# sakdag/multimodal-misinformation-detection

Measured on AMD Instinct MI355X. Metric: claim–evidence pairs/sec (fwd+bwd) at bs=256; 1/2/4/8 MI355X scaling, higher is better.
Workload: dtype fp32; 1 GPU; full fine-tune bert-base-uncased + ViT-B/16 + fusion head (768/768, E=256, H=8), fwd+bwd+AdamW; global_batch=256, seq_len=128, image_size=224, parallelism=dp1

## Files before the change

multimodal-misinformation-detection_amd/csrc/attention.hip:

```cpp
#include "attn_common.h"
#include "attn_stream.h"
#include "attn_resident.h"
#include "attn_split.h"
#include <algorithm>
#include <initializer_list>
#include <stdio.h>
#include <stdlib.h>
#include <string.h>

namespace {

int g_v2_generic = [] {
  const char* v = getenv("MMFD_ATTN_V2_GENERIC");
  return v && atoi(v) != 0 ? 1 : 0;
}();

const bool g_attn_v1 = getenv("MMFD_ATTN_V1") != nullptr;

int g_fp32_attn_mode = [] {
  const char* v = getenv("MMFD_FP32_ATTN");
  const char* gm = getenv("MMFD_FP32_GEMM");
  const bool native = (v && (!strcmp(v, "native") || !strcmp(v, "0"))) ||
                      (!v && gm && (!strcmp(gm, "native") || !strcmp(gm, "0")));
  return native ? 0 : 1;
}();

const int g_x6a_dbg = getenv("MMFD_X6A_DBG") ? atoi(getenv("MMFD_X6A_DBG")) : 0;

int fill(const mmfd_attn_args& a, AttnP& p, bool bwd) {
  MMFD_CHECK_ARG(a.dtype == MMFD_F32 || a.dtype == MMFD_BF16, "attn: bad dtype");
  MMFD_CHECK_ARG(a.D > 0 && a.D <= 64, "attn: head_dim %lld unsupported (<= 64)", (long long)a.D);
  MMFD_CHECK_ARG(a.B >= 0 && a.H > 0 && a.Lq >= 0 && a.Lk > 0, "attn: bad shape");
  MMFD_CHECK_ARG(a.q && a.k && a.v && a.o && a.lse, "attn: null pointer");
  const int epc = a.dtype == MMFD_BF16 ? 8 : 4;
  MMFD_CHECK_ARG(a.D % epc == 0, "attn: head_dim*element_size must be a multiple of 16 bytes");
  auto al = [&](const void* ptr, int64_t sb, int64_t st) {
    return ((uintptr_t)ptr & 15) == 0 && sb % epc == 0 && st % epc == 0;
  };
  MMFD_CHECK_ARG(al(a.q, a.q_sb, a.q_st) && al(a.k, a.k_sb, a.k_st) && al(a.v, a.v_sb, a.v_st),
                 "attn: q/k/v must be 16-B aligned with strides multiple of 16 B");
  MMFD_CHECK_ARG(a.dropout_p <= 0.f || a.seed, "attn: dropout needs seed");
  MMFD_CHECK_ARG(a.dropout_p < 1.f, "attn: dropout p must be < 1");
  if (bwd) {
    MMFD_CHECK_ARG(a.dout && a.dq && a.dk && a.dv && a.delta, "attn_bwd: null pointer");
    MMFD_CHECK_ARG(al(a.dout, a.do_sb, a.do_st), "attn_bwd: dout alignment");
    if (a.d_rel_bias) {
      MMFD_CHECK_ARG(a.rel_bias && a.rel_bias_sb == a.H * a.Lq * a.Lk && a.rel_bias_mod == 0,
                     "attn_bwd: d_rel_bias needs a per-batch rel_bias [B][H][Lq][Lk] (rel_bias_sb = H*Lq*Lk, rel_bias_mod = 0)");
// ... 83 lines not shown
  return KERN_TD(attn_fwd_v2_kernel, HPB, false, 0);
}

template <typename T, int D, bool REL, int MODE>
void add_bwd_v2(Plan& pl, AttnP& p, const char* what) {
  constexpr int NTH = V2T<T>::DKDV_THREADS;
  const int lq_pad = v2_pad(p.Lq, v2_kc<T>()), lk_pad = v2_pad(p.Lk, v2_kc<T>());
  constexpr int dkdv_max = v2_dkdv_lds<T, D>(V2_LMAX, V2_LMAX / 32);
  p.dm_lds = p.p > 0.f && p.dm && v2_dkdv_lds<T, D>(lq_pad, p.dmw) <= dkdv_max;
  const dim3 heads((unsigned)(p.B * p.H));
  pl.add(KERN_TD(attn_dq_v2_kernel, REL, MODE), heads, V2_THREADS, v2_dq_lds<T, D>(lk_pad), v2_dq_lds<T, D>(V2_LMAX), what);
  pl.add(KERN_TD(attn_dkdv_v2_kernel, NTH, REL, MODE), heads, NTH, v2_dkdv_lds<T, D>(lq_pad, p.dm_lds ? p.dmw : 0),
         dkdv_max, what);
}

template <typename T, int D>
void plan_kernels(Plan& pl, AttnP& p, const mmfd_attn_args& a, bool bwd) {
  const char* what = bwd ? "attn_bwd" : "attn_fwd";
  const int64_t nbh = p.B * p.H;
  const dim3 heads((unsigned)nbh);
  const dim3 qblocks((unsigned)((p.Lq + 63) / 64), (unsigned)nbh), kblocks((unsigned)((p.Lk + 63) / 64), (unsigned)nbh);
  if (pl.family == SPLIT) {
    const int lq16 = v2_pad(p.Lq, 16), lk16 = v2_pad(p.Lk, 16);
    if (!bwd) {
      pl.add(p.p > 0.f ? KERN_D(attn_fwd_x6_kernel, true) : KERN_D(attn_fwd_x6_kernel, false), heads, V2_THREADS,
             x6_kv_lds(lk16), X6A_LDS, what);
    } else {
      const int dqd = p.p <= 0.f ? 0 : !p.dm ? 1 : 2;
      const int dkd = dqd == 2 && x6_dkdv_lds(lq16, lk16, p.dmw) > X6A_LDS_MAX ? 1 : dqd;
      pl.add(dqd == 0 ? KERN_D(attn_dq_x6_kernel, 0) : dqd == 1 ? KERN_D(attn_dq_x6_kernel, 1) : KERN_D(attn_dq_x6_kernel, 2),
             heads, V2_THREADS, x6_kv_lds(lk16), X6A_LDS, what);
      pl.add(dkd == 0 ? KERN_D(attn_dkdv_x6_kernel, 0) : dkd == 1 ? KERN_D(attn_dkdv_x6_kernel, 1) : KERN_D(attn_dkdv_x6_kernel, 2),
             heads, V2_THREADS, x6_dkdv_lds(lq16, lk16, dkd == 2 ? p.dmw : 0), X6A_LDS_MAX, what);
    }
  } else if (pl.family == RESIDENT && !bwd) {
    const int hpb = p.Lk <= 64 && p.Lq <= 32 ? 4 : p.Lk <= 64 && p.Lq <= 64 ? 2 : 1;
    const int lmax = hpb > 1 ? 64 : sizeof(T) == 2 ? V2_LMAX_FWD : V2_LMAX;
    pl.add(hpb == 4 ? fwd_v2_kern<T, D, 4>(p) : hpb == 2 ? fwd_v2_kern<T, D, 2>(p) : fwd_v2_kern<T, D, 1>(p),
           dim3((unsigned)((nbh + hpb - 1) / hpb)), V2_THREADS,
           v2_fwd_lds<T, D>(hpb, v2_pad(p.Lk, v2_kc<T>())) + (p.cos_ls ? v2_fwd_cos_lds(hpb, v2_pad(p.Lk, v2_kc<T>())) : 0),
           v2_fwd_lds<T, D>(hpb, lmax) + v2_fwd_cos_lds(hpb, lmax), what);
  } else if (pl.family == RESIDENT) {
    const int mode = v2_mode(p);
    if (p.rel_bias) add_bwd_v2<T, D, true, 0>(pl, p, what);
    else if (mode == 1) add_bwd_v2<T, D, false, 1>(pl, p, what);
    else if (mode == 2) add_bwd_v2<T, D, false, 2>(pl, p, what);
    else add_bwd_v2<T, D, false, 0>(pl, p, what);
  } else if (!bwd) {
    pl.add(KERN_TD(attn_fwd_kernel), qblocks, 256, stream_kv_lds<T, D>(), 0, what);
  } else {
    const int64_t threads = nbh * p.Lq * AT<T, D>::NCH;
    pl.add(KERN_TD(attn_delta_kernel), dim3((unsigned)((threads + 255) / 256)), 256, 0, 0, what);
    pl.add(KERN_TD(attn_bwd_dkdv_kernel), kblocks, 256, stream_dkdv_lds<T, D>(), 0, what);
    pl.add(KERN_TD(attn_bwd_dq_kernel), qblocks, 256, stream_dq_lds<T, D>(), 0, what);
// ... 92 lines not shown
    const Step& st = pl.step[i];
    put("%s", st.k.name);
    for (int j = 0; j < st.k.narg; ++j) {
      if (j == 0) put("%s", st.k.bf < 0 ? "<" : st.k.bf ? "<bf16," : "<float,");
      put(j + 1 < st.k.narg ? "%d," : "%d>", st.k.arg[j]);
    }
    put(" grid=%u,%u,%u block=%u lds=%d%s%s%s%s%s%s", st.grid.x, st.grid.y, st.grid.z, st.block, st.lds,
        p.pl ? " pl" : "", p.pl_only ? " pl_only" : "", p.vst ? " vst" : "", p.dm ? " dm" : "",
        p.dm_lds ? " dm_lds" : "", p.idx32 ? " idx32" : "");
    if (p.pl) put(" pl_stride=%lld", (long long)p.pl_stride);
    put("%s", "\n");
  }
  if (pl.split3) put("mmfd_split3 rows=%lld W=%lld\n", (long long)(p.B * p.Lq), (long long)((bwd ? 3 : 1) * a->H * a->D));
  MMFD_CHECK_ARG(at < bytes, "mmfd_debug_attn_plan: buffer of %lld bytes is too small", (long long)bytes);
  return 0;
}

extern "C" int mmfd_debug_set_attn_v2_generic(int on) {
  const int old = g_v2_generic;
  g_v2_generic = on ? 1 : 0;
  return old;
}

extern "C" int mmfd_set_fp32_attn_mode(int mode) {
  MMFD_CHECK_ARG(mode == 0 || mode == 1, "mmfd_set_fp32_attn_mode: mode %d (0 = fp32 MFMA, 1 = split operands)", mode);
  const int old = g_fp32_attn_mode;
  g_fp32_attn_mode = mode;
  return old;
}

#ifdef MMFD_X6A_STAMPS
extern "C" int mmfd_debug_x6a_stamps(void* host_dst, int64_t bytes) {
  return (int)hipMemcpyFromSymbol(host_dst, HIP_SYMBOL(x6a_stamps), (size_t)bytes, 0, hipMemcpyDeviceToHost);
}
#endif
```

multimodal-misinformation-detection_amd/csrc/attn_split.h:

```cpp
#pragma once
#include "attn_resident.h"

namespace {


#ifdef MMFD_X6A_STAMPS
__device__ uint64_t x6a_stamps[8192 * 8 * 16];
#define X6A_STAMP(k)                                                                               \
  do {                                                                                             \
    const uint64_t t__ = __builtin_amdgcn_s_memtime();                                             \
    if (lane == 0 && blockIdx.x < 8192) x6a_stamps[((int64_t)blockIdx.x * 8 + wave) * 16 + (k)] = t__; \
  } while (0)
#else
#define X6A_STAMP(k) do { } while (0)
#endif
constexpr int X6A_LMAX = 208;
constexpr int X6A_RB = 128;
constexpr int X6A_LDS = 6 * X6A_LMAX * X6A_RB + 3 * X6A_LMAX * 4;
constexpr int X6A_LDS_MAX = 160 * 1024;
constexpr int x6_kv_lds(int lk16) { return 6 * lk16 * X6A_RB + lk16 * 4; }
constexpr int x6_dkdv_lds(int lq16, int lk16, int dm_words) {
  return 6 * lq16 * X6A_RB + (2 * lq16 + lk16) * 4 + lq16 * dm_words * 4;
}

__device__ __forceinline__ void split8(const float* x, uint4& hi, uint4& mid, uint4& lo) {
  bf16x8 h, m, l;
#pragma unroll
  for (int u = 0; u < 8; ++u) {
    const bf16 hu = (bf16)x[u];
    const float r = x[u] - (float)hu;
    const bf16 mu = (bf16)r;
    h[u] = hu;
    m[u] = mu;
    l[u] = (bf16)(r - (float)mu);
// ... 15 lines not shown

__device__ __forceinline__ void split_acc(const f32x4& a, const f32x4& b, uint4& hi, uint4& mid, uint4& lo) {
  const float x[8] = {a[0], a[1], a[2], a[3], b[0], b[1], b[2], b[3]};
  split8(x, hi, mid, lo);
}

template <int KCH> struct X6Row { float4 v[KCH][2]; };
template <int KCH>
__device__ __forceinline__ void x6_row_load(X6Row<KCH>& x, const float* __restrict__ base, int64_t st, int64_t row,
                                            int64_t nrows, int lane, int dreal) {
  const int g = lane >> 4;
#pragma unroll
  for (int kc = 0; kc < KCH; ++kc) {
    const int col = (kc * 4 + g) * 8;
    x.v[kc][0] = x.v[kc][1] = make_float4(0.f, 0.f, 0.f, 0.f);
    if (row < nrows && col < dreal) {
      const float* src = base + row * st + col;
      x.v[kc][0] = *reinterpret_cast<const float4*>(src);
      x.v[kc][1] = *reinterpret_cast<const float4*>(src + 4);
    }
  }
}
template <int KCH>
__device__ __forceinline__ void x6_row_split(uint4 (&f)[3][KCH], const X6Row<KCH>& x) {
#pragma unroll
  for (int kc = 0; kc < KCH; ++kc) {
    const float4 a = x.v[kc][0], b = x.v[kc][1];
    const float e[8] = {a.x, a.y, a.z, a.w, b.x, b.y, b.z, b.w};
    split8(e, f[0][kc], f[1][kc], f[2][kc]);
  }
}

template <int D, int NTH>
__device__ __forceinline__ void x6_stage2(char* img_a, const float* __restrict__ base_a, int64_t st_a, char* img_b,
                                          const float* __restrict__ base_b, int64_t st_b, int img, int64_t nrows,
                                          int nrows_pad, int tid, int dreal, int dbg) {
  constexpr int NC = D / 8;
  constexpr int MAXT = (X6A_LMAX * NC + NTH - 1) / NTH;
  const int total = nrows_pad * NC;
  float4 xa[MAXT][2], xb[MAXT][2];
#pragma unroll
  for (int j = 0; j < MAXT; ++j) {
    const int c = tid + j * NTH;
    const int r = c / NC, ch = c % NC;
    xa[j][0] = xa[j][1] = xb[j][0] = xb[j][1] = make_float4(0.f, 0.f, 0.f, 0.f);
    if (c < total && r < nrows && ch * 8 < dreal && !(dbg & 1)) {
      const float* sa = base_a + (int64_t)r * st_a + ch * 8;
      const float* sb = base_b + (int64_t)r * st_b + ch * 8;
      xa[j][0] = *reinterpret_cast<const float4*>(sa);
      xa[j][1] = *reinterpret_cast<const float4*>(sa + 4);
      xb[j][0] = *reinterpret_cast<const float4*>(sb);
      xb[j][1] = *reinterpret_cast<const float4*>(sb + 4);
    }
  }
#pragma unroll
  for (int j = 0; j < MAXT; ++j) {
    const int c = tid + j * NTH;
    if (c < total) {
      const int r = c / NC, ch = c % NC;
      const int off = row_off<bf16, 64>(r, ch);
      uint4 h, m, l;
      {
        const float e[8] = {xa[j][0].x, xa[j][0].y, xa[j][0].z, xa[j][0].w, xa[j][1].x, xa[j][1].y, xa[j][1].z, xa[j][1].w};
        split8(e, h, m, l);
        *reinterpret_cast<uint4*>(img_a + off) = h;
        *reinterpret_cast<uint4*>(img_a + img + off) = m;
        *reinterpret_cast<uint4*>(img_a + 2 * img + off) = l;
      }
      {
        const float e[8] = {xb[j][0].x, xb[j][0].y, xb[j][0].z, xb[j][0].w, xb[j][1].x, xb[j][1].y, xb[j][1].z, xb[j][1].w};
        split8(e, h, m, l);
        *reinterpret_cast<uint4*>(img_b + off) = h;
        *reinterpret_cast<uint4*>(img_b + img + off) = m;
        *reinterpret_cast<uint4*>(img_b + 2 * img + off) = l;
      }
    }
  }
}

__device__ __forceinline__ uint4 x6_tr_frag(const char* lds, int c, int dsub, int lane, int h1off) {
  const int g = lane >> 4, i = lane & 15, q = i >> 2;
  const int u = dsub * 4 + (i & 3);
  const int r = c * 32 + 4 * g + q;
  const int off = r * X6A_RB + (((u >> 1) ^ (r & 7)) << 4) + ((u & 1) << 3);
  const uint2 x0 = lds_read_tr16(lds + off);
  const uint2 x1 = lds_read_tr16(lds + off + h1off);
  return make_uint4(x0.x, x0.y, x1.x, x1.y);
}

__device__ __forceinline__ void x6_row_frag3(uint4* f, const char* lds, int img, int sub, int kc, int lane) {
  f[0] = row_frag<bf16, 64>(lds, sub, kc, lane);
  f[1] = row_frag<bf16, 64>(lds + img, sub, kc, lane);
  f[2] = row_frag<bf16, 64>(lds + 2 * img, sub, kc, lane);
}
__device__ __forceinline__ void x6_tr_frag3(uint4* f, const char* lds, int img, int c, int d, int lane, int h1off) {
  f[0] = x6_tr_frag(lds, c, d, lane, h1off);
  f[1] = x6_tr_frag(lds + img, c, d, lane, h1off);
  f[2] = x6_tr_frag(lds + 2 * img, c, d, lane, h1off);
}


template <int D, bool DROP>
__global__ void __launch_bounds__(V2_THREADS, 1) attn_fwd_x6_kernel(AttnP p) {
  constexpr int KCH = D / 32, DT = D / 16;
  extern __shared__ __attribute__((aligned(16))) char smem[];
  const int tid = threadIdx.x, lane = tid & 63, g = lane >> 4, li = lane & 15;
  const int wave = __builtin_amdgcn_readfirstlane(tid >> 6);
  const int64_t bh = blockIdx.x, b = bh / p.H, h = bh % p.H;
  X6A_STAMP(0);
  const int lk16 = v2_pad(p.Lk, 16);
  const int img = lk16 * X6A_RB;
  char* k_img = smem;
  char* v_img = smem + 3 * img;
  float* kbias = reinterpret_cast<float*>(smem + 6 * img);
  const float* qb = reinterpret_cast<const float*>(p.q) + b * p.q_sb + h * p.D;
  X6Row<KCH> qn;
  x6_row_load<KCH>(qn, qb, p.q_st, (int64_t)wave * 16 + li, p.Lq, lane, p.D);
  x6_stage2<D, V2_THREADS>(k_img, reinterpret_cast<const float*>(p.k) + b * p.k_sb + h * p.D, p.k_st, v_img,
                           reinterpret_cast<const float*>(p.v) + b * p.v_sb + h * p.D, p.v_st, img, p.Lk, lk16, tid,
                           p.D, p.dbg);
  stage_kbias<V2_THREADS>(kbias, p, b, lk16, tid);
  __syncthreads();
  X6A_STAMP(1);
  const uint64_t seed = DROP ? *p.seed : 0ull;
  const uint32_t hkey = mmfd_hash_key(seed, p.salt);
  const float c2 = p.scale * LOG2E;
  float* ob = reinterpret_cast<float*>(p.o) + b * p.o_sb + h * p.D;
  const int nqb = (int)((p.Lq + 15) / 16);
  const int nfc = lk16 / 64;
  const int nchk = nfc + ((lk16 & 63) ? 1 : 0);
  auto qrun = [&](int qbk, const uint4 (&qf)[3][KCH], int c0, int c1, f32x4 (&o)[DT], float& m, float& lsum) {
// ... 101 lines not shown
  auto qfin = [&](int qbk, const f32x4 (&o)[DT], float m, float lsum) {
    const int64_t q0 = (int64_t)qbk * 16, myq = q0 + li;
#pragma unroll
    for (int r = 0; r < 4; ++r) {
      const float lr = __shfl(lsum, 4 * g + r, 64);
      const int64_t q = q0 + 4 * g + r;
      const float inv = 1.0f / lr;
      if (q < p.Lq) {
#pragma unroll
        for (int d = 0; d < DT; ++d)
          if (d * 16 + li < p.D) {
            const float val = o[d][r] * inv;
            ob[q * p.o_st + d * 16 + li] = val;
            if (p.pl) plane_put(p, ob + q * p.o_st + d * 16 + li, val);
          }
      }
    }
    if (g == 0 && myq < p.Lq) p.lse[bh * p.Lq + myq] = (m + log2f(lsum)) * LN2;
  };
  if (p.dbg & 2) return;
  const int R = nqb - V2_THREADS / 64;
  const bool split = R >= 1 && R <= V2_THREADS / 64 && (R & 3) == 1 && nchk >= 2;
  const int nwhole = split ? nqb - 1 : nqb;
  for (int qbk = wave; qbk < nwhole; qbk += V2_THREADS / 64) {
    uint4 qf[3][KCH];
    x6_row_split<KCH>(qf, qn);
    if (qbk + V2_THREADS / 64 < nwhole)
      x6_row_load<KCH>(qn, qb, p.q_st, (int64_t)(qbk + V2_THREADS / 64) * 16 + li, p.Lq, lane, p.D);
    if (qbk == wave) X6A_STAMP(2);
    float m = -INFINITY, lsum = 0.f;
    f32x4 o[DT];
#pragma unroll
    for (int d = 0; d < DT; ++d) o[d] = f32x4{0.f, 0.f, 0.f, 0.f};
    qrun(qbk, qf, 0, nchk, o, m, lsum);
    if (qbk == wave) X6A_STAMP(7);
    lsum += __shfl_xor(lsum, 16, 64);
    lsum += __shfl_xor(lsum, 32, 64);
    qfin(qbk, o, m, lsum);
    if (qbk == wave) X6A_STAMP(8);
  }
  if (split) {
    const int sb = nqb - 1, hc = nchk / 2;
    const bool own = wave == R - 1, part = wave == R;
    float m = -INFINITY, lsum = 0.f;
    f32x4 o[DT];
#pragma unroll
    for (int d = 0; d < DT; ++d) o[d] = f32x4{0.f, 0.f, 0.f, 0.f};
    if (own || part) {
      X6Row<KCH> qr;
      x6_row_load<KCH>(qr, qb, p.q_st, (int64_t)sb * 16 + li, p.Lq, lane, p.D);
      uint4 qf[3][KCH];
      x6_row_split<KCH>(qf, qr);
      qrun(sb, qf, own ? 0 : hc, own ? hc : nchk, o, m, lsum);
      lsum += __shfl_xor(lsum, 16, 64);
      lsum += __shfl_xor(lsum, 32, 64);
    }
    __syncthreads();
    f32x4* xo = reinterpret_cast<f32x4*>(smem);
    float* xm = reinterpret_cast<float*>(smem + DT * 64 * 16);
    if (part) {
#pragma unroll
      for (int d = 0; d < DT; ++d) xo[d * 64 + lane] = o[d];
      xm[lane] = m;
      xm[64 + lane] = lsum;
    }
    __syncthreads();
    if (own) {
      const float mb = xm[lane], lb = xm[64 + lane];
      const float mm = fmaxf(m, mb);
      const float aa = __builtin_amdgcn_exp2f(m - mm), ab = __builtin_amdgcn_exp2f(mb - mm);
#pragma unroll
      for (int r = 0; r < 4; ++r) {
        const float ra = __shfl(aa, 4 * g + r, 64), rb = __shfl(ab, 4 * g + r, 64);
#pragma unroll
        for (int d = 0; d < DT; ++d) o[d][r] = o[d][r] * ra + xo[d * 64 + lane][r] * rb;
      }
      qfin(sb, o, mm, lsum * aa + lb * ab);
    }
  }
  X6A_STAMP(9);
}

template <int D, int DROP>
__global__ void __launch_bounds__(V2_THREADS, 1) attn_dkdv_x6_kernel(AttnP p) {
  constexpr int KCH = D / 32, DT = D / 16;
  extern __shared__ __attribute__((aligned(16))) char smem[];
  const int tid = threadIdx.x, lane = tid & 63, g = lane >> 4, li = lane & 15;
  const int wave = __builtin_amdgcn_readfirstlane(tid >> 6);
  const int64_t bh = blockIdx.x, b = bh / p.H, h = bh % p.H;
  const int lq16 = v2_pad(p.Lq, 16), lk16 = v2_pad(p.Lk, 16);
  const int img = lq16 * X6A_RB;
  char* q_img = smem;
  char* do_img = smem + 3 * img;
  float* s_lse = reinterpret_cast<float*>(smem + 6 * img);
  float* s_delta = s_lse + lq16;
  float* kbias = s_delta + lq16;
  uint32_t* s_dm = reinterpret_cast<uint32_t*>(kbias + lk16);
  const float* kb = reinterpret_cast<const float*>(p.k) + b * p.k_sb + h * p.D;
  const float* vb = reinterpret_cast<const float*>(p.v) + b * p.v_sb + h * p.D;
  if constexpr (DROP == 2) {
    const uint32_t* src = dm_row(p, bh, 0);
    const int nw = (int)p.Lq * p.dmw;
    for (int i = tid; i < lq16 * p.dmw; i += V2_THREADS) s_dm[i] = i < nw ? src[i] : 0u;
  }
// ... 180 lines not shown
#pragma unroll
    for (int i = 0; i < 2 * DT; ++i) dkv[i] = f32x4{0.f, 0.f, 0.f, 0.f};
    if (own || part) {
      X6Row<KCH> kr, vr;
      x6_row_load<KCH>(kr, kb, p.k_st, (int64_t)sb * 16 + li, p.Lk, lane, p.D);
      x6_row_load<KCH>(vr, vb, p.v_st, (int64_t)sb * 16 + li, p.Lk, lane, p.D);
      kblock(sb, kr, vr, own ? 0 : hc, own ? hc : nch, dkv);
    }
    __syncthreads();
    f32x4* xch = reinterpret_cast<f32x4*>(smem);
    if (part) {
#pragma unroll
      for (int i = 0; i < 2 * DT; ++i) xch[i * 64 + lane] = dkv[i];
    }
    __syncthreads();
    if (own) {
#pragma unroll
      for (int i = 0; i < 2 * DT; ++i) dkv[i] += xch[i * 64 + lane];
      kstore(sb, dkv);
    }
  }
}

template <int D, int DROP>
__global__ void __launch_bounds__(V2_THREADS, 1) attn_dq_x6_kernel(AttnP p) {
  constexpr int KCH = D / 32, DT = D / 16;
  extern __shared__ __attribute__((aligned(16))) char smem[];
  const int tid = threadIdx.x, lane = tid & 63, g = lane >> 4, li = lane & 15;
  const int wave = __builtin_amdgcn_readfirstlane(tid >> 6);
  const int64_t bh = blockIdx.x, b = bh / p.H, h = bh % p.H;
  const int lk16 = v2_pad(p.Lk, 16);
  const int img = lk16 * X6A_RB;
  char* k_img = smem;
  char* v_img = smem + 3 * img;
  float* kbias = reinterpret_cast<float*>(smem + 6 * img);
  const float* qb = reinterpret_cast<const float*>(p.q) + b * p.q_sb + h * p.D;
  const float* dob = reinterpret_cast<const float*>(p.dout) + b * p.do_sb + h * p.D;
  const float* obp = reinterpret_cast<const float*>(p.o) + b * p.o_sb + h * p.D;
  X6Row<KCH> qn, don, on;
  x6_row_load<KCH>(qn, qb, p.q_st, (int64_t)wave * 16 + li, p.Lq, lane, p.D);
  x6_row_load<KCH>(don, dob, p.do_st, (int64_t)wave * 16 + li, p.Lq, lane, p.D);
  x6_row_load<KCH>(on, obp, p.o_st, (int64_t)wave * 16 + li, p.Lq, lane, p.D);
  x6_stage2<D, V2_THREADS>(k_img, reinterpret_cast<const float*>(p.k) + b * p.k_sb + h * p.D, p.k_st, v_img,
                           reinterpret_cast<const float*>(p.v) + b * p.v_sb + h * p.D, p.v_st, img, p.Lk, lk16, tid,
                           p.D, p.dbg);
  stage_kbias<V2_THREADS>(kbias, p, b, lk16, tid);
  __syncthreads();
  float* dqb = reinterpret_cast<float*>(p.dq) + b * p.dq_sb + h * p.D;
  const uint64_t seed = DROP ? *p.seed : 0ull;
  const uint32_t hkey = mmfd_hash_key(seed, p.salt);
  const float c2 = p.scale * LOG2E;
  const int nqb = (int)((p.Lq + 15) / 16);
  auto qblock = [&](int qbk, const X6Row<KCH>& qr, const X6Row<KCH>& dr, const X6Row<KCH>& orow, bool wdelta,
                    int ka, int kb2e, f32x4 (&dq)[DT]) {
    const int64_t q0 = (int64_t)qbk * 16, myq = q0 + li;
    uint4 qf[3][KCH], dof[3][KCH];
    x6_row_split<KCH>(qf, qr);
    x6_row_split<KCH>(dof, dr);
    const float lse2 = myq < p.Lq ? p.lse[bh * p.Lq + myq] * LOG2E : INFINITY;
    float dsum = 0.f;
#pragma unroll
    for (int kc = 0; kc < KCH; ++kc)
#pragma unroll
      for (int hh = 0; hh < 2; ++hh) {
        const float4 a = orow.v[kc][hh], c = dr.v[kc][hh];
        dsum = fmaf(a.x, c.x, fmaf(a.y, c.y, fmaf(a.z, c.z, fmaf(a.w, c.w, dsum))));
      }
    dsum += __shfl_xor(dsum, 16, 64);
    dsum += __shfl_xor(dsum, 32, 64);
    const float dlt = myq < p.Lq ? dsum : 0.f;
    if (wdelta && g == 0 && myq < p.Lq) p.delta[bh * p.Lq + myq] = dsum;
    const uint64_t hrow = (uint64_t)(bh * p.Lq + myq) * (uint64_t)p.kp;
    const uint32_t rowc1 = ((uint32_t)hrow + (uint32_t)(2 * g)) * HASH_C1;
    const uint32_t* dmrow = DROP == 2 ? dm_row(p, bh, myq < p.Lq ? myq : 0) : nullptr;
    auto chunk = [&](int kc2, auto nsc) {
      constexpr int NS = decltype(nsc)::value;
      uint32_t kw = 0;
      if constexpr (DROP == 2) kw = dmrow[kc2];
      f32x4 sd[4];
#pragma unroll
      for (int i = 0; i < 4; ++i) sd[i] = f32x4{0.f, 0.f, 0.f, 0.f};
      {
// ... 81 lines not shown
    for (int r = 0; r < 4; ++r) {
      const int64_t q = q0 + 4 * g + r;
      if (q < p.Lq) {
#pragma unroll
        for (int d = 0; d < DT; ++d) {
          if (d * 16 + li >= p.D) continue;
          float* pq = dqb + q * p.dq_st + d * 16 + li;
          float vq = dq[d][r] * p.scale;
          if (p.acc_dq) vq += *pq;
          if (p.pl) {
            plane_put(p, pq, vq);
            if (p.pl_only) continue;
          }
          *pq = vq;
        }
      }
    }
  };
  if (p.dbg & 2) return;
  const int nch = lk16 / 32 + ((lk16 & 16) ? 1 : 0);
  const int R = nqb - V2_THREADS / 64;
  const bool split = R >= 1 && R <= V2_THREADS / 64 && (R & 3) == 1 && nch >= 2;
  const int nwhole = split ? nqb - 1 : nqb;
  if (wave < nwhole) {
    f32x4 dq[DT];
#pragma unroll
    for (int d = 0; d < DT; ++d) dq[d] = f32x4{0.f, 0.f, 0.f, 0.f};
    qblock(wave, qn, don, on, true, 0, nch, dq);
    qstore(wave, dq);
  }
  for (int qbk = wave + V2_THREADS / 64; qbk < nwhole; qbk += V2_THREADS / 64) {
    X6Row<KCH> qr, dr, orr;
    x6_row_load<KCH>(qr, qb, p.q_st, (int64_t)qbk * 16 + li, p.Lq, lane, p.D);
    x6_row_load<KCH>(dr, dob, p.do_st, (int64_t)qbk * 16 + li, p.Lq, lane, p.D);
    x6_row_load<KCH>(orr, obp, p.o_st, (int64_t)qbk * 16 + li, p.Lq, lane, p.D);
    f32x4 dq[DT];
#pragma unroll
    for (int d = 0; d < DT; ++d) dq[d] = f32x4{0.f, 0.f, 0.f, 0.f};
    qblock(qbk, qr, dr, orr, true, 0, nch, dq);
    qstore(qbk, dq);
  }
  if (split) {
    const int sb = nqb - 1, hc = nch / 2;
    const bool own = wave == R - 1, part = wave == R;
    f32x4 dq[DT];
#pragma unroll
    for (int d = 0; d < DT; ++d) dq[d] = f32x4{0.f, 0.f, 0.f, 0.f};
    if (own || part) {
      X6Row<KCH> qr, dr, orr;
      x6_row_load<KCH>(qr, qb, p.q_st, (int64_t)sb * 16 + li, p.Lq, lane, p.D);
      x6_row_load<KCH>(dr, dob, p.do_st, (int64_t)sb * 16 + li, p.Lq, lane, p.D);
      x6_row_load<KCH>(orr, obp, p.o_st, (int64_t)sb * 16 + li, p.Lq, lane, p.D);
      qblock(sb, qr, dr, orr, own, own ? 0 : hc, own ? hc : nch, dq);
    }
    __syncthreads();
    f32x4* xch = reinterpret_cast<f32x4*>(smem);
    if (part) {
#pragma unroll
      for (int d = 0; d < DT; ++d) xch[d * 64 + lane] = dq[d];
    }
    __syncthreads();
    if (own) {
#pragma unroll
      for (int d = 0; d < DT; ++d) dq[d] += xch[d * 64 + lane];
      qstore(sb, dq);
    }
  }
}
}
```

Measured before the change: 590.8 pairs/s.

## Add persistent x6 attention fwd/dq kernels that prefetch the next head's K/V

Adds persistent variants of the split-operand fp32 attention forward and dQ kernels. A fixed grid of up to 256 workgroups walks the batch×head list, and each walker prefetches the next head's K/V, key bias and first Q/dO/O rows into registers while it computes the current head. At a barrier it then splits the prefetched data into the LDS images. This is meant to hide global-load latency and per-block launch/staging cost when there are many heads. It is enabled by default when nbh is at least 1024, and is selectable per Lk via templates. The cost is higher register pressure and extra barriers, with the risk of lower parallelism if there are too few walkers.

```diff
diff --git a/multimodal-misinformation-detection_amd/csrc/attention.hip b/multimodal-misinformation-detection_amd/csrc/attention.hip
--- a/multimodal-misinformation-detection_amd/csrc/attention.hip
+++ b/multimodal-misinformation-detection_amd/csrc/attention.hip
@@ -4,6 +4,7 @@
 #include "attn_split.h"
 #include <algorithm>
 #include <initializer_list>
+#include <stdint.h>
 #include <stdio.h>
 #include <stdlib.h>
 #include <string.h>
@@ -24,6 +25,16 @@
                       (!v && gm && (!strcmp(gm, "native") || !strcmp(gm, "0")));
   return native ? 0 : 1;
 }();
+
+constexpr int X6P_WGS = 256;
+constexpr int64_t X6P_MIN_HEADS = 4 * X6P_WGS;
+constexpr int64_t X6P_MAX_HEADS = 65536;
+constexpr int64_t X6P_OFF = INT64_MAX;
+int64_t g_x6p_min_heads = [] {
+  const char* v = getenv("MMFD_ATTN_X6_PERSIST");
+  return v && atoi(v) == 0 ? X6P_OFF : X6P_MIN_HEADS;
+}();
+int g_x6p_wgs = X6P_WGS;
 
 const int g_x6a_dbg = getenv("MMFD_X6A_DBG") ? atoi(getenv("MMFD_X6A_DBG")) : 0;
 
@@ -153,14 +164,30 @@
   const dim3 qblocks((unsigned)((p.Lq + 63) / 64), (unsigned)nbh), kblocks((unsigned)((p.Lk + 63) / 64), (unsigned)nbh);
   if (pl.family == SPLIT) {
     const int lq16 = v2_pad(p.Lq, 16), lk16 = v2_pad(p.Lk, 16);
-    if (!bwd) {
+    const bool persist = nbh >= g_x6p_min_heads && nbh <= X6P_MAX_HEADS;
+    const bool small = lk16 <= 128;
+    const dim3 walkers((unsigned)std::min<int64_t>(nbh, g_x6p_wgs));
+    if (!bwd && persist && small) {
+      pl.add(p.p > 0.f ? KERN_D(attn_fwd_x6p_kernel, true, 128) : KERN_D(attn_fwd_x6p_kernel, false, 128), walkers,
+             V2_THREADS, x6_kv_lds(lk16), X6A_LDS, what);
+    } else if (!bwd) {
       pl.add(p.p > 0.f ? KERN_D(attn_fwd_x6_kernel, true) : KERN_D(attn_fwd_x6_kernel, false), heads, V2_THREADS,
              x6_kv_lds(lk16), X6A_LDS, what);
     } else {
       const int dqd = p.p <= 0.f ? 0 : !p.dm ? 1 : 2;
       const int dkd = dqd == 2 && x6_dkdv_lds(lq16, lk16, p.dmw) > X6A_LDS_MAX ? 1 : dqd;
-      pl.add(dqd == 0 ? KERN_D(attn_dq_x6_kernel, 0) : dqd == 1 ? KERN_D(attn_dq_x6_kernel, 1) : KERN_D(attn_dq_x6_kernel, 2),
-             heads, V2_THREADS, x6_kv_lds(lk16), X6A_LDS, what);
+      if (persist && small)
+        pl.add(dqd == 0 ? KERN_D(attn_dq_x6p_kernel, 0, 128) : dqd == 1 ? KERN_D(attn_dq_x6p_kernel, 1, 128)
+                                                                        : KERN_D(attn_dq_x6p_kernel, 2, 128),
+               walkers, V2_THREADS, x6_kv_lds(lk16), X6A_LDS, what);
+      else if (persist)
+        pl.add(dqd == 0 ? KERN_D(attn_dq_x6p_kernel, 0, X6A_LMAX) : dqd == 1 ? KERN_D(attn_dq_x6p_kernel, 1, X6A_LMAX)
+                                                                             : KERN_D(attn_dq_x6p_kernel, 2, X6A_LMAX),
+               walkers, V2_THREADS, x6_kv_lds(lk16), X6A_LDS, what);
+      else
+        pl.add(dqd == 0 ? KERN_D(attn_dq_x6_kernel, 0) : dqd == 1 ? KERN_D(attn_dq_x6_kernel, 1)
+                                                                 : KERN_D(attn_dq_x6_kernel, 2),
+               heads, V2_THREADS, x6_kv_lds(lk16), X6A_LDS, what);
       pl.add(dkd == 0 ? KERN_D(attn_dkdv_x6_kernel, 0) : dkd == 1 ? KERN_D(attn_dkdv_x6_kernel, 1) : KERN_D(attn_dkdv_x6_kernel, 2),
              heads, V2_THREADS, x6_dkdv_lds(lq16, lk16, dkd == 2 ? p.dmw : 0), X6A_LDS_MAX, what);
     }
@@ -299,6 +326,15 @@
   return old;
 }
 
+extern "C" int mmfd_debug_set_attn_x6_persist(int64_t min_heads, int wgs, int64_t* old_min_heads, int* old_wgs) {
+  MMFD_CHECK_ARG(wgs >= 1, "mmfd_debug_set_attn_x6_persist: wgs %d (>= 1)", wgs);
+  if (old_min_heads) *old_min_heads = g_x6p_min_heads == X6P_OFF ? 0 : g_x6p_min_heads;
+  if (old_wgs) *old_wgs = g_x6p_wgs;
+  g_x6p_min_heads = min_heads <= 0 ? X6P_OFF : min_heads;
+  g_x6p_wgs = wgs;
+  return 0;
+}
+
 extern "C" int mmfd_set_fp32_attn_mode(int mode) {
   MMFD_CHECK_ARG(mode == 0 || mode == 1, "mmfd_set_fp32_attn_mode: mode %d (0 = fp32 MFMA, 1 = split operands)", mode);
   const int old = g_fp32_attn_mode;
diff --git a/multimodal-misinformation-detection_amd/csrc/attn_split.h b/multimodal-misinformation-detection_amd/csrc/attn_split.h
--- a/multimodal-misinformation-detection_amd/csrc/attn_split.h
+++ b/multimodal-misinformation-detection_amd/csrc/attn_split.h
@@ -9,7 +9,7 @@
 #define X6A_STAMP(k)                                                                               \
   do {                                                                                             \
     const uint64_t t__ = __builtin_amdgcn_s_memtime();                                             \
-    if (lane == 0 && blockIdx.x < 8192) x6a_stamps[((int64_t)blockIdx.x * 8 + wave) * 16 + (k)] = t__; \
+    if (lane == 0 && bh < 8192) x6a_stamps[(bh * 8 + wave) * 16 + (k)] = t__;                      \
   } while (0)
 #else
 #define X6A_STAMP(k) do { } while (0)
@@ -71,6 +71,25 @@
   }
 }
 template <int KCH>
+__device__ __forceinline__ void x6_row_load_ahead(X6Row<KCH>& x, const float* __restrict__ base, int64_t st,
+                                                  int64_t row, int64_t nrows, int lane, int dreal) {
+  const int g = lane >> 4;
+#pragma unroll
+  for (int kc = 0; kc < KCH; ++kc) {
+    const int col = (kc * 4 + g) * 8;
+    const float* src = base + (row < nrows && col < dreal ? row * st + col : 0);
+    x.v[kc][0] = *reinterpret_cast<const float4*>(src);
+    x.v[kc][1] = *reinterpret_cast<const float4*>(src + 4);
+  }
+}
+template <int KCH>
+__device__ __forceinline__ void x6_row_mask(X6Row<KCH>& x, int64_t row, int64_t nrows, int lane, int dreal) {
+  const int g = lane >> 4;
+#pragma unroll
+  for (int kc = 0; kc < KCH; ++kc)
+    if (!(row < nrows && (kc * 4 + g) * 8 < dreal)) x.v[kc][0] = x.v[kc][1] = make_float4(0.f, 0.f, 0.f, 0.f);
+}
+template <int KCH>
 __device__ __forceinline__ void x6_row_split(uint4 (&f)[3][KCH], const X6Row<KCH>& x) {
 #pragma unroll
   for (int kc = 0; kc < KCH; ++kc) {
@@ -80,51 +99,90 @@
   }
 }
 
+template <int D, int NTH> constexpr int x6_stage_depth(int rows) { return (rows * (D / 8) + NTH - 1) / NTH; }
+template <int NJ> struct X6Stage { float4 a[NJ][2], b[NJ][2]; };
+template <int D, int NTH, int NJ, bool TWO, bool AHEAD = false>
+__device__ __forceinline__ void x6_stage_load(X6Stage<NJ>& x, const float* __restrict__ base_a, int64_t st_a,
+                                              const float* __restrict__ base_b, int64_t st_b, int64_t nrows,
+                                              int nrows_pad, int tid, int dreal, int dbg) {
+  constexpr int NC = D / 8;
+  const int total = nrows_pad * NC;
+#pragma unroll
+  for (int j = 0; j < NJ; ++j) {
+    const int c = tid + j * NTH;
+    const int r = c / NC, ch = c % NC;
+    if constexpr (AHEAD) {
+      const bool ok = c < total && r < nrows && ch * 8 < dreal;
+      const float* sa = base_a + (ok ? (int64_t)r * st_a + ch * 8 : 0);
+      x.a[j][0] = *reinterpret_cast<const float4*>(sa);
+      x.a[j][1] = *reinterpret_cast<const float4*>(sa + 4);
+      if constexpr (TWO) {
+        const float* sb = base_b + (ok ? (int64_t)r * st_b + ch * 8 : 0);
+        x.b[j][0] = *reinterpret_cast<const float4*>(sb);
+        x.b[j][1] = *reinterpret_cast<const float4*>(sb + 4);
+      }
+      continue;
+    }
+    x.a[j][0] = x.a[j][1] = make_float4(0.f, 0.f, 0.f, 0.f);
+    if constexpr (TWO) x.b[j][0] = x.b[j][1] = make_float4(0.f, 0.f, 0.f, 0.f);
+    if (c < total && r < nrows && ch * 8 < dreal && !(dbg & 1)) {
+      const float* sa = base_a + (int64_t)r * st_a + ch * 8;
+      x.a[j][0] = *reinterpret_cast<const float4*>(sa);
+      x.a[j][1] = *reinterpret_cast<const float4*>(sa + 4);
+      if constexpr (TWO) {
+        const float* sb = base_b + (int64_t)r * st_b + ch * 8;
+        x.b[j][0] = *reinterpret_cast<const float4*>(sb);
+        x.b[j][1] = *reinterpret_cast<const float4*>(sb + 4);
+      }
+    }
+  }
+}
+template <int D, int NTH, int NJ, bool TWO, bool AHEAD = false>
+__device__ __forceinline__ void x6_stage_split(char* img_a, char* img_b, int img, const X6Stage<NJ>& x, int nrows_pad,
+                                               int tid, int64_t nrows = 0, int dreal = 0, int dbg = 0) {
+  constexpr int NC = D / 8;
+  const int total = nrows_pad * NC;
+#pragma unroll
+  for (int j = 0; j < NJ; ++j) {
+    const int c = tid + j * NTH;
+    if (c < total) {
+      const int r = c / NC, ch = c % NC;
+      const int off = row_off<bf16, 64>(r, ch);
+      const bool zero = AHEAD && !(r < nrows && ch * 8 < dreal && !(dbg & 1));
+      uint4 h, m, l;
+      {
+        float4 a0 = x.a[j][0], a1 = x.a[j][1];
+        if constexpr (AHEAD) {
+          if (zero) a0 = a1 = make_float4(0.f, 0.f, 0.f, 0.f);
+        }
+        const float e[8] = {a0.x, a0.y, a0.z, a0.w, a1.x, a1.y, a1.z, a1.w};
+        split8(e, h, m, l);
+        *reinterpret_cast<uint4*>(img_a + off) = h;
+        *reinterpret_cast<uint4*>(img_a + img + off) = m;
+        *reinterpret_cast<uint4*>(img_a + 2 * img + off) = l;
+      }
+      if constexpr (TWO) {
+        float4 b0 = x.b[j][0], b1 = x.b[j][1];
+        if constexpr (AHEAD) {
+          if (zero) b0 = b1 = make_float4(0.f, 0.f, 0.f, 0.f);
+        }
+        const float e[8] = {b0.x, b0.y, b0.z, b0.w, b1.x, b1.y, b1.z, b1.w};
+        split8(e, h, m, l);
+        *reinterpret_cast<uint4*>(img_b + off) = h;
+        *reinterpret_cast<uint4*>(img_b + img + off) = m;
+        *reinterpret_cast<uint4*>(img_b + 2 * img + off) = l;
+      }
+    }
+  }
+}
 template <int D, int NTH>
 __device__ __forceinline__ void x6_stage2(char* img_a, const float* __restrict__ base_a, int64_t st_a, char* img_b,
                                           const float* __restrict__ base_b, int64_t st_b, int img, int64_t nrows,
                                           int nrows_pad, int tid, int dreal, int dbg) {
-  constexpr int NC = D / 8;
-  constexpr int MAXT = (X6A_LMAX * NC + NTH - 1) / NTH;
-  const int total = nrows_pad * NC;
-  float4 xa[MAXT][2], xb[MAXT][2];
-#pragma unroll
-  for (int j = 0; j < MAXT; ++j) {
-    const int c = tid + j * NTH;
-    const int r = c / NC, ch = c % NC;
-    xa[j][0] = xa[j][1] = xb[j][0] = xb[j][1] = make_float4(0.f, 0.f, 0.f, 0.f);
-    if (c < total && r < nrows && ch * 8 < dreal && !(dbg & 1)) {
-      const float* sa = base_a + (int64_t)r * st_a + ch * 8;
-      const float* sb = base_b + (int64_t)r * st_b + ch * 8;
-      xa[j][0] = *reinterpret_cast<const float4*>(sa);
-      xa[j][1] = *reinterpret_cast<const float4*>(sa + 4);
-      xb[j][0] = *reinterpret_cast<const float4*>(sb);
-      xb[j][1] = *reinterpret_cast<const float4*>(sb + 4);
-    }
-  }
-#pragma unroll
-  for (int j = 0; j < MAXT; ++j) {
-    const int c = tid + j * NTH;
-    if (c < total) {
-      const int r = c / NC, ch = c % NC;
-      const int off = row_off<bf16, 64>(r, ch);
-      uint4 h, m, l;
-      {
-        const float e[8] = {xa[j][0].x, xa[j][0].y, xa[j][0].z, xa[j][0].w, xa[j][1].x, xa[j][1].y, xa[j][1].z, xa[j][1].w};
-        split8(e, h, m, l);
-        *reinterpret_cast<uint4*>(img_a + off) = h;
-        *reinterpret_cast<uint4*>(img_a + img + off) = m;
-        *reinterpret_cast<uint4*>(img_a + 2 * img + off) = l;
-      }
-      {
-        const float e[8] = {xb[j][0].x, xb[j][0].y, xb[j][0].z, xb[j][0].w, xb[j][1].x, xb[j][1].y, xb[j][1].z, xb[j][1].w};
-        split8(e, h, m, l);
-        *reinterpret_cast<uint4*>(img_b + off) = h;
-        *reinterpret_cast<uint4*>(img_b + img + off) = m;
-        *reinterpret_cast<uint4*>(img_b + 2 * img + off) = l;
-      }
-    }
-  }
+  constexpr int NJ = x6_stage_depth<D, NTH>(X6A_LMAX);
+  X6Stage<NJ> x;
+  x6_stage_load<D, NTH, NJ, true>(x, base_a, st_a, base_b, st_b, nrows, nrows_pad, tid, dreal, dbg);
+  x6_stage_split<D, NTH, NJ, true>(img_a, img_b, img, x, nrows_pad, tid);
 }
 
 __device__ __forceinline__ uint4 x6_tr_frag(const char* lds, int c, int dsub, int lane, int h1off) {
@@ -149,13 +207,45 @@
 }
 
 
-template <int D, bool DROP>
-__global__ void __launch_bounds__(V2_THREADS, 1) attn_fwd_x6_kernel(AttnP p) {
+template <int D, int LC> struct X6P {
+  static constexpr int NJ = x6_stage_depth<D, V2_THREADS>(LC ? LC : X6A_LMAX);
+  static constexpr bool V = NJ <= 2;
+};
+__device__ __forceinline__ int x6p_fresh(int v) {
+  asm volatile("" : "+v"(v));
+  return v;
+}
+__device__ __forceinline__ float x6_kbias_load(const AttnP& p, int64_t b, int tid) {
+  return p.key_bias ? p.key_bias[b * p.Lk + (tid < p.Lk ? tid : 0)] : 0.f;
+}
+template <int D, int LC>
+__device__ __forceinline__ void x6p_boundary(char* k_img, char* v_img, float* kbias, int img,
+                                             X6Stage<X6P<D, LC>::NJ>& x, float kbn, const float* __restrict__ vbase,
+                                             const AttnP& p, int lk16, int tid) {
+  constexpr int NJ = X6P<D, LC>::NJ;
+  tid = x6p_fresh(tid);
+  asm volatile("" : "+v"(kbn));
+  __syncthreads();
+  if constexpr (X6P<D, LC>::V) {
+    x6_stage_split<D, V2_THREADS, NJ, true, true>(k_img, v_img, img, x, lk16, tid, p.Lk, p.D, p.dbg);
+  } else {
+    X6Stage<NJ> y;
+    x6_stage_load<D, V2_THREADS, NJ, false>(y, vbase, p.v_st, nullptr, 0, p.Lk, lk16, tid, p.D, p.dbg);
+    x6_stage_split<D, V2_THREADS, NJ, false, true>(k_img, nullptr, img, x, lk16, tid, p.Lk, p.D, p.dbg);
+    x6_stage_split<D, V2_THREADS, NJ, false>(v_img, nullptr, img, y, lk16, tid);
+  }
+  if (tid < lk16) kbias[tid] = tid < p.Lk ? (p.key_bias ? fmaxf(kbn * LOG2E, -1e30f) : 0.f) : -INFINITY;
+  __syncthreads();
+}
+
+template <int D, bool DROP, int LC>
+__device__ __forceinline__ void x6_fwd_heads(const AttnP& p) {
   constexpr int KCH = D / 32, DT = D / 16;
+  constexpr bool PERSIST = LC != 0;
   extern __shared__ __attribute__((aligned(16))) char smem[];
-  const int tid = threadIdx.x, lane = tid & 63, g = lane >> 4, li = lane & 15;
+  int tid = threadIdx.x, lane = tid & 63, g = lane >> 4, li = lane & 15;
   const int wave = __builtin_amdgcn_readfirstlane(tid >> 6);
-  const int64_t bh = blockIdx.x, b = bh / p.H, h = bh % p.H;
+  int64_t bh = blockIdx.x, b = bh / p.H, h = bh % p.H;
   X6A_STAMP(0);
   const int lk16 = v2_pad(p.Lk, 16);
   const int img = lk16 * X6A_RB;
@@ -303,64 +393,103 @@
   const int R = nqb - V2_THREADS / 64;
   const bool split = R >= 1 && R <= V2_THREADS / 64 && (R & 3) == 1 && nchk >= 2;
   const int nwhole = split ? nqb - 1 : nqb;
-  for (int qbk = wave; qbk < nwhole; qbk += V2_THREADS / 64) {
-    uint4 qf[3][KCH];
-    x6_row_split<KCH>(qf, qn);
-    if (qbk + V2_THREADS / 64 < nwhole)
-      x6_row_load<KCH>(qn, qb, p.q_st, (int64_t)(qbk + V2_THREADS / 64) * 16 + li, p.Lq, lane, p.D);
-    if (qbk == wave) X6A_STAMP(2);
-    float m = -INFINITY, lsum = 0.f;
-    f32x4 o[DT];
-#pragma unroll
-    for (int d = 0; d < DT; ++d) o[d] = f32x4{0.f, 0.f, 0.f, 0.f};
-    qrun(qbk, qf, 0, nchk, o, m, lsum);
-    if (qbk == wave) X6A_STAMP(7);
-    lsum += __shfl_xor(lsum, 16, 64);
-    lsum += __shfl_xor(lsum, 32, 64);
-    qfin(qbk, o, m, lsum);
-    if (qbk == wave) X6A_STAMP(8);
-  }
-  if (split) {
-    const int sb = nqb - 1, hc = nchk / 2;
-    const bool own = wave == R - 1, part = wave == R;
-    float m = -INFINITY, lsum = 0.f;
-    f32x4 o[DT];
-#pragma unroll
-    for (int d = 0; d < DT; ++d) o[d] = f32x4{0.f, 0.f, 0.f, 0.f};
-    if (own || part) {
-      X6Row<KCH> qr;
-      x6_row_load<KCH>(qr, qb, p.q_st, (int64_t)sb * 16 + li, p.Lq, lane, p.D);
+  for (;;) {
+    X6Stage<X6P<D, LC>::NJ> kvn;
+    float kbn = 0.f;
+    int64_t nbh = 0, nb = 0, nh = 0;
+    bool more = false;
+    if constexpr (PERSIST) {
+      tid = x6p_fresh(tid), lane = tid & 63, g = lane >> 4, li = lane & 15;
+      nbh = bh + gridDim.x;
+      more = nbh < p.B * p.H;
+      nb = nbh / p.H, nh = nbh % p.H;
+    }
+    auto ahead = [&]() {
+      if (more) {
+        const int t = x6p_fresh(tid);
+        x6_stage_load<D, V2_THREADS, X6P<D, LC>::NJ, X6P<D, LC>::V, true>(
+            kvn, reinterpret_cast<const float*>(p.k) + nb * p.k_sb + nh * p.D, p.k_st,
+            reinterpret_cast<const float*>(p.v) + nb * p.v_sb + nh * p.D, p.v_st, p.Lk, lk16, t, p.D, p.dbg);
+        kbn = x6_kbias_load(p, nb, t);
+      }
+    };
+    if (PERSIST && wave >= nwhole) ahead();
+    for (int qbk = wave; qbk < nwhole; qbk += V2_THREADS / 64) {
       uint4 qf[3][KCH];
-      x6_row_split<KCH>(qf, qr);
-      qrun(sb, qf, own ? 0 : hc, own ? hc : nchk, o, m, lsum);
+      x6_row_split<KCH>(qf, qn);
+      if (qbk + V2_THREADS / 64 < nwhole)
+        x6_row_load<KCH>(qn, qb, p.q_st, (int64_t)(qbk + V2_THREADS / 64) * 16 + li, p.Lq, lane, p.D);
+      else if (PERSIST && more)
+        x6_row_load<KCH>(qn, reinterpret_cast<const float*>(p.q) + nb * p.q_sb + nh * p.D, p.q_st,
+                         (int64_t)wave * 16 + li, p.Lq, lane, p.D);
+      if (PERSIST && qbk == wave) ahead();
+      if (qbk == wave) X6A_STAMP(2);
+      float m = -INFINITY, lsum = 0.f;
+      f32x4 o[DT];
+#pragma unroll
+      for (int d = 0; d < DT; ++d) o[d] = f32x4{0.f, 0.f, 0.f, 0.f};
+      qrun(qbk, qf, 0, nchk, o, m, lsum);
+      if (qbk == wave) X6A_STAMP(7);
       lsum += __shfl_xor(lsum, 16, 64);
       lsum += __shfl_xor(lsum, 32, 64);
-    }
-    __syncthreads();
-    f32x4* xo = reinterpret_cast<f32x4*>(smem);
-    float* xm = reinterpret_cast<float*>(smem + DT * 64 * 16);
-    if (part) {
-#pragma unroll
-      for (int d = 0; d < DT; ++d) xo[d * 64 + lane] = o[d];
-      xm[lane] = m;
-      xm[64 + lane] = lsum;
-    }
-    __syncthreads();
-    if (own) {
-      const float mb = xm[lane], lb = xm[64 + lane];
-      const float mm = fmaxf(m, mb);
-      const float aa = __builtin_amdgcn_exp2f(m - mm), ab = __builtin_amdgcn_exp2f(mb - mm);
-#pragma unroll
-      for (int r = 0; r < 4; ++r) {
-        const float ra = __shfl(aa, 4 * g + r, 64), rb = __shfl(ab, 4 * g + r, 64);
-#pragma unroll
-        for (int d = 0; d < DT; ++d) o[d][r] = o[d][r] * ra + xo[d * 64 + lane][r] * rb;
-      }
-      qfin(sb, o, mm, lsum * aa + lb * ab);
-    }
-  }
-  X6A_STAMP(9);
-}
+      qfin(qbk, o, m, lsum);
+      if (qbk == wave) X6A_STAMP(8);
+    }
+    if (split) {
+      const int sb = nqb - 1, hc = nchk / 2;
+      const bool own = wave == R - 1, part = wave == R;
+      float m = -INFINITY, lsum = 0.f;
+      f32x4 o[DT];
+#pragma unroll
+      for (int d = 0; d < DT; ++d) o[d] = f32x4{0.f, 0.f, 0.f, 0.f};
+      if (own || part) {
+        X6Row<KCH> qr;
+        x6_row_load<KCH>(qr, qb, p.q_st, (int64_t)sb * 16 + li, p.Lq, lane, p.D);
+        uint4 qf[3][KCH];
+        x6_row_split<KCH>(qf, qr);
+        qrun(sb, qf, own ? 0 : hc, own ? hc : nchk, o, m, lsum);
+        lsum += __shfl_xor(lsum, 16, 64);
+        lsum += __shfl_xor(lsum, 32, 64);
+      }
+      __syncthreads();
+      f32x4* xo = reinterpret_cast<f32x4*>(smem);
+      float* xm = reinterpret_cast<float*>(smem + DT * 64 * 16);
+      if (part) {
+#pragma unroll
+        for (int d = 0; d < DT; ++d) xo[d * 64 + lane] = o[d];
+        xm[lane] = m;
+        xm[64 + lane] = lsum;
+      }
+      __syncthreads();
+      if (own) {
+        const float mb = xm[lane], lb = xm[64 + lane];
+        const float mm = fmaxf(m, mb);
+        const float aa = __builtin_amdgcn_exp2f(m - mm), ab = __builtin_amdgcn_exp2f(mb - mm);
+#pragma unroll
+        for (int r = 0; r < 4; ++r) {
+          const float ra = __shfl(aa, 4 * g + r, 64), rb = __shfl(ab, 4 * g + r, 64);
+#pragma unroll
+          for (int d = 0; d < DT; ++d) o[d][r] = o[d][r] * ra + xo[d * 64 + lane][r] * rb;
+        }
+        qfin(sb, o, mm, lsum * aa + lb * ab);
+      }
+    }
+    X6A_STAMP(9);
+    if (!PERSIST || !more) break;
+    bh = nbh, b = nb, h = nh;
+    qb = reinterpret_cast<const float*>(p.q) + b * p.q_sb + h * p.D;
+    ob = reinterpret_cast<float*>(p.o) + b * p.o_sb + h * p.D;
+    X6A_STAMP(0);
+    x6p_boundary<D, LC>(k_img, v_img, kbias, img, kvn, kbn,
+                        reinterpret_cast<const float*>(p.v) + b * p.v_sb + h * p.D, p, lk16, tid);
+    X6A_STAMP(1);
+  }
+}
+
+template <int D, bool DROP>
+__global__ void __launch_bounds__(V2_THREADS, 1) attn_fwd_x6_kernel(AttnP p) { x6_fwd_heads<D, DROP, 0>(p); }
+template <int D, bool DROP, int LC>
+__global__ void __launch_bounds__(V2_THREADS, 1) attn_fwd_x6p_kernel(AttnP p) { x6_fwd_heads<D, DROP, LC>(p); }
 
 template <int D, int DROP>
 __global__ void __launch_bounds__(V2_THREADS, 1) attn_dkdv_x6_kernel(AttnP p) {
@@ -587,13 +716,14 @@
   }
 }
 
-template <int D, int DROP>
-__global__ void __launch_bounds__(V2_THREADS, 1) attn_dq_x6_kernel(AttnP p) {
+template <int D, int DROP, int LC>
+__device__ __forceinline__ void x6_dq_heads(const AttnP& p) {
   constexpr int KCH = D / 32, DT = D / 16;
+  constexpr bool PERSIST = LC != 0;
   extern __shared__ __attribute__((aligned(16))) char smem[];
-  const int tid = threadIdx.x, lane = tid & 63, g = lane >> 4, li = lane & 15;
+  int tid = threadIdx.x, lane = tid & 63, g = lane >> 4, li = lane & 15;
   const int wave = __builtin_amdgcn_readfirstlane(tid >> 6);
-  const int64_t bh = blockIdx.x, b = bh / p.H, h = bh % p.H;
+  int64_t bh = blockIdx.x, b = bh / p.H, h = bh % p.H;
   const int lk16 = v2_pad(p.Lk, 16);
   const int img = lk16 * X6A_RB;
   char* k_img = smem;
@@ -603,26 +733,36 @@
   const float* dob = reinterpret_cast<const float*>(p.dout) + b * p.do_sb + h * p.D;
   const float* obp = reinterpret_cast<const float*>(p.o) + b * p.o_sb + h * p.D;
   X6Row<KCH> qn, don, on;
-  x6_row_load<KCH>(qn, qb, p.q_st, (int64_t)wave * 16 + li, p.Lq, lane, p.D);
-  x6_row_load<KCH>(don, dob, p.do_st, (int64_t)wave * 16 + li, p.Lq, lane, p.D);
-  x6_row_load<KCH>(on, obp, p.o_st, (int64_t)wave * 16 + li, p.Lq, lane, p.D);
-  x6_stage2<D, V2_THREADS>(k_img, reinterpret_cast<const float*>(p.k) + b * p.k_sb + h * p.D, p.k_st, v_img,
-                           reinterpret_cast<const float*>(p.v) + b * p.v_sb + h * p.D, p.v_st, img, p.Lk, lk16, tid,
-                           p.D, p.dbg);
-  stage_kbias<V2_THREADS>(kbias, p, b, lk16, tid);
-  __syncthreads();
+  X6Stage<X6P<D, LC>::NJ> kvn;
+  float kbn = 0.f, lse1 = 0.f;
+  if constexpr (!PERSIST) {
+    x6_row_load<KCH>(qn, qb, p.q_st, (int64_t)wave * 16 + li, p.Lq, lane, p.D);
+    x6_row_load<KCH>(don, dob, p.do_st, (int64_t)wave * 16 + li, p.Lq, lane, p.D);
+    x6_row_load<KCH>(on, obp, p.o_st, (int64_t)wave * 16 + li, p.Lq, lane, p.D);
+    x6_stage2<D, V2_THREADS>(k_img, reinterpret_cast<const float*>(p.k) + b * p.k_sb + h * p.D, p.k_st, v_img,
+                             reinterpret_cast<const float*>(p.v) + b * p.v_sb + h * p.D, p.v_st, img, p.Lk, lk16, tid,
+                             p.D, p.dbg);
+    stage_kbias<V2_THREADS>(kbias, p, b, lk16, tid);
+    __syncthreads();
+  } else {
+    x6_stage_load<D, V2_THREADS, X6P<D, LC>::NJ, X6P<D, LC>::V, true>(
+        kvn, reinterpret_cast<const float*>(p.k) + b * p.k_sb + h * p.D, p.k_st,
+        reinterpret_cast<const float*>(p.v) + b * p.v_sb + h * p.D, p.v_st, p.Lk, lk16, tid, p.D, p.dbg);
+    kbn = x6_kbias_load(p, b, tid);
+  }
   float* dqb = reinterpret_cast<float*>(p.dq) + b * p.dq_sb + h * p.D;
   const uint64_t seed = DROP ? *p.seed : 0ull;
   const uint32_t hkey = mmfd_hash_key(seed, p.salt);
   const float c2 = p.scale * LOG2E;
   const int nqb = (int)((p.Lq + 15) / 16);
   auto qblock = [&](int qbk, const X6Row<KCH>& qr, const X6Row<KCH>& dr, const X6Row<KCH>& orow, bool wdelta,
-                    int ka, int kb2e, f32x4 (&dq)[DT]) {
+                    int ka, int kb2e, f32x4 (&dq)[DT], auto firstc) {
+    constexpr bool first = PERSIST && decltype(firstc)::value;
     const int64_t q0 = (int64_t)qbk * 16, myq = q0 + li;
     uint4 qf[3][KCH], dof[3][KCH];
     x6_row_split<KCH>(qf, qr);
     x6_row_split<KCH>(dof, dr);
-    const float lse2 = myq < p.Lq ? p.lse[bh * p.Lq + myq] * LOG2E : INFINITY;
+    const float lse2 = myq < p.Lq ? (first ? lse1 : p.lse[bh * p.Lq + myq]) * LOG2E : INFINITY;
     float dsum = 0.f;
 #pragma unroll
     for (int kc = 0; kc < KCH; ++kc)
@@ -750,49 +890,87 @@
   const int R = nqb - V2_THREADS / 64;
   const bool split = R >= 1 && R <= V2_THREADS / 64 && (R & 3) == 1 && nch >= 2;
   const int nwhole = split ? nqb - 1 : nqb;
-  if (wave < nwhole) {
-    f32x4 dq[DT];
-#pragma unroll
-    for (int d = 0; d < DT; ++d) dq[d] = f32x4{0.f, 0.f, 0.f, 0.f};
-    qblock(wave, qn, don, on, true, 0, nch, dq);
-    qstore(wave, dq);
-  }
-  for (int qbk = wave + V2_THREADS / 64; qbk < nwhole; qbk += V2_THREADS / 64) {
-    X6Row<KCH> qr, dr, orr;
-    x6_row_load<KCH>(qr, qb, p.q_st, (int64_t)qbk * 16 + li, p.Lq, lane, p.D);
-    x6_row_load<KCH>(dr, dob, p.do_st, (int64_t)qbk * 16 + li, p.Lq, lane, p.D);
-    x6_row_load<KCH>(orr, obp, p.o_st, (int64_t)qbk * 16 + li, p.Lq, lane, p.D);
-    f32x4 dq[DT];
-#pragma unroll
-    for (int d = 0; d < DT; ++d) dq[d] = f32x4{0.f, 0.f, 0.f, 0.f};
-    qblock(qbk, qr, dr, orr, true, 0, nch, dq);
-    qstore(qbk, dq);
-  }
-  if (split) {
-    const int sb = nqb - 1, hc = nch / 2;
-    const bool own = wave == R - 1, part = wave == R;
-    f32x4 dq[DT];
-#pragma unroll
-    for (int d = 0; d < DT; ++d) dq[d] = f32x4{0.f, 0.f, 0.f, 0.f};
-    if (own || part) {
+  for (;;) {
+    int64_t nbh = 0, nb = 0, nh = 0;
+    bool more = false;
+    if constexpr (PERSIST) {
+      tid = x6p_fresh(tid), lane = tid & 63, g = lane >> 4, li = lane & 15;
+      const int64_t row1 = (int64_t)wave * 16 + li;
+      x6_row_load_ahead<KCH>(qn, qb, p.q_st, row1, p.Lq, lane, p.D);
+      x6_row_load_ahead<KCH>(don, dob, p.do_st, row1, p.Lq, lane, p.D);
+      x6_row_load_ahead<KCH>(on, obp, p.o_st, row1, p.Lq, lane, p.D);
+      lse1 = p.lse[bh * p.Lq + (row1 < p.Lq ? row1 : 0)];
+      x6p_boundary<D, LC>(k_img, v_img, kbias, img, kvn, kbn,
+                          reinterpret_cast<const float*>(p.v) + b * p.v_sb + h * p.D, p, lk16, tid);
+      x6_row_mask<KCH>(qn, row1, p.Lq, lane, p.D);
+      x6_row_mask<KCH>(don, row1, p.Lq, lane, p.D);
+      x6_row_mask<KCH>(on, row1, p.Lq, lane, p.D);
+      asm volatile("" : "+v"(lse1));
+      nbh = bh + gridDim.x;
+      more = nbh < p.B * p.H;
+      nb = nbh / p.H, nh = nbh % p.H;
+      if (more) {
+        x6_stage_load<D, V2_THREADS, X6P<D, LC>::NJ, X6P<D, LC>::V, true>(
+            kvn, reinterpret_cast<const float*>(p.k) + nb * p.k_sb + nh * p.D, p.k_st,
+            reinterpret_cast<const float*>(p.v) + nb * p.v_sb + nh * p.D, p.v_st, p.Lk, lk16, tid, p.D, p.dbg);
+        kbn = x6_kbias_load(p, nb, tid);
+      }
+    }
+    if (wave < nwhole) {
+      f32x4 dq[DT];
+#pragma unroll
+      for (int d = 0; d < DT; ++d) dq[d] = f32x4{0.f, 0.f, 0.f, 0.f};
+      qblock(wave, qn, don, on, true, 0, nch, dq, std::true_type{});
+      qstore(wave, dq);
+    }
+    for (int qbk = wave + V2_THREADS / 64; qbk < nwhole; qbk += V2_THREADS / 64) {
       X6Row<KCH> qr, dr, orr;
-      x6_row_load<KCH>(qr, qb, p.q_st, (int64_t)sb * 16 + li, p.Lq, lane, p.D);
-      x6_row_load<KCH>(dr, dob, p.do_st, (int64_t)sb * 16 + li, p.Lq, lane, p.D);
-      x6_row_load<KCH>(orr, obp, p.o_st, (int64_t)sb * 16 + li, p.Lq, lane, p.D);
-      qblock(sb, qr, dr, orr, own, own ? 0 : hc, own ? hc : nch, dq);
-    }
-    __syncthreads();
-    f32x4* xch = reinterpret_cast<f32x4*>(smem);
-    if (part) {
-#pragma unroll
-      for (int d = 0; d < DT; ++d) xch[d * 64 + lane] = dq[d];
-    }
-    __syncthreads();
-    if (own) {
-#pragma unroll
-      for (int d = 0; d < DT; ++d) dq[d] += xch[d * 64 + lane];
-      qstore(sb, dq);
-    }
-  }
-}
-}
+      x6_row_load<KCH>(qr, qb, p.q_st, (int64_t)qbk * 16 + li, p.Lq, lane, p.D);
+      x6_row_load<KCH>(dr, dob, p.do_st, (int64_t)qbk * 16 + li, p.Lq, lane, p.D);
+      x6_row_load<KCH>(orr, obp, p.o_st, (int64_t)qbk * 16 + li, p.Lq, lane, p.D);
+      f32x4 dq[DT];
+#pragma unroll
+      for (int d = 0; d < DT; ++d) dq[d] = f32x4{0.f, 0.f, 0.f, 0.f};
+      qblock(qbk, qr, dr, orr, true, 0, nch, dq, std::false_type{});
+      qstore(qbk, dq);
+    }
+    if (split) {
+      const int sb = nqb - 1, hc = nch / 2;
+      const bool own = wave == R - 1, part = wave == R;
+      f32x4 dq[DT];
+#pragma unroll
+      for (int d = 0; d < DT; ++d) dq[d] = f32x4{0.f, 0.f, 0.f, 0.f};
+      if (own || part) {
+        X6Row<KCH> qr, dr, orr;
+        x6_row_load<KCH>(qr, qb, p.q_st, (int64_t)sb * 16 + li, p.Lq, lane, p.D);
+        x6_row_load<KCH>(dr, dob, p.do_st, (int64_t)sb * 16 + li, p.Lq, lane, p.D);
+        x6_row_load<KCH>(orr, obp, p.o_st, (int64_t)sb * 16 + li, p.Lq, lane, p.D);
+        qblock(sb, qr, dr, orr, own, own ? 0 : hc, own ? hc : nch, dq, std::false_type{});
+      }
+      __syncthreads();
+      f32x4* xch = reinterpret_cast<f32x4*>(smem);
+      if (part) {
+#pragma unroll
+        for (int d = 0; d < DT; ++d) xch[d * 64 + lane] = dq[d];
+      }
+      __syncthreads();
+      if (own) {
+#pragma unroll
+        for (int d = 0; d < DT; ++d) dq[d] += xch[d * 64 + lane];
+        qstore(sb, dq);
+      }
+    }
+    if (!PERSIST || !more) break;
+    bh = nbh, b = nb, h = nh;
+    qb = reinterpret_cast<const float*>(p.q) + b * p.q_sb + h * p.D;
+    dob = reinterpret_cast<const float*>(p.dout) + b * p.do_sb + h * p.D;
+    obp = reinterpret_cast<const float*>(p.o) + b * p.o_sb + h * p.D;
+    dqb = reinterpret_cast<float*>(p.dq) + b * p.dq_sb + h * p.D;
+  }
+}
+
+template <int D, int DROP>
+__global__ void __launch_bounds__(V2_THREADS, 1) attn_dq_x6_kernel(AttnP p) { x6_dq_heads<D, DROP, 0>(p); }
+template <int D, int DROP, int LC>
+__global__ void __launch_bounds__(V2_THREADS, 1) attn_dq_x6p_kernel(AttnP p) { x6_dq_heads<D, DROP, LC>(p); }
+}
```

Result: no change. 590.8 pairs/s (median of 5 runs) (-0.0%).
